# ivanacollg/MPC_CollisionAvoidance

Measured on AMD Instinct MI355X. Metric: batched SQP-RTI solves/sec (USV, N=40 horizon, 10 obstacles), higher is better.
Workload: dtype f64

## Files before the change

mpc_collisionavoidance_amd/csrc/params.hpp:

```cpp
#pragma once

namespace usv {

constexpr int LANES = 16;
constexpr int KMAX = 32;

struct DevSpec {
    double Hc[LANES * LANES];
    double He[LANES * LANES];
    double Mc[LANES * LANES];
    double Me[LANES * LANES];
    double lb[LANES], ub[LANES];
    int has_b[LANES];
    int boxpack;
    int boxpack_ok;
    int box_dense;
    int aux_dense4;
    int box_slot[LANES];
    int box_step[LANES];
    int slot_var[LANES];
    int slot_is[LANES];
    double uh[KMAX];
    double lsl[KMAX], lsu[KMAX];
    double zl[KMAX], zu[KMAX], Zl[KMAX], Zu[KMAX];
// ... 96 lines not shown
    double *u;
    const double *x0;
    const double *yref;
    const double *yref_e;
    const double *p;
    const double *lh;
    double *sl, *su;
    double *pi;
    int *status;
    int *qp_iter;
    int *qp_status;
    double *res;
    double *obs_tmin;
    int *fail_count;
    double *nlp_res;
    int *sqp_iter;
    int *sqp_state;
    int *sqp_running;
    double *ws;
    int *queue;
    int *epoch;
    int *redo;
    int redo_words;
    const int *perm_cur;
    const int *inv_next;
    int tick;
    double *lam_out, *t_out;
    int nlam;
    int *susp_count;
    int *susp_list;
    double *susp_rec;
    int handover_iter;
    int *co_ctl;
};

}
```

mpc_collisionavoidance_amd/csrc/qp_ipm.hpp:

```cpp
#pragma once
#include "lanes.hpp"
#include "params.hpp"
#include "sfor.hpp"

#pragma clang fp contract(on)

namespace usv {

template <bool SOFTROW, bool MIXED = false>
struct RowCalc {
    double ll, lu, tl, tu, sl, su, lsl, lsu, tsl, tsu;
    double dl, du, zl, zu, Zl, Zu, bsl, bsu;
    bool act, soft;
    double rdl, rdu, rsl, rsu, rdsl, rdsu;
    USV_DEV bool is_soft() const
    {
        if constexpr (!SOFTROW) return false;
        else if constexpr (MIXED) return soft;
        else return true;
    }
    double itl, itu, itsl, itsu;
    double Gl, Gu, iDl, iDu, rhol, rhou;
    double ml, mu, msl, msu;
    double dll, dlu, dtl, dtu, dsl, dsu, dlsl, dlsu, dtsl, dtsu;

    USV_DEV void neutral()
    {
        ll = lu = 0.0; tl = tu = 1.0; sl = su = 0.0; lsl = lsu = 0.0; tsl = tsu = 1.0;
        dl = -1.0; du = 1.0; zl = zu = 0.0; Zl = Zu = 1.0; bsl = bsu = -1.0;
        soft = SOFTROW && !MIXED;
    }
    USV_DEV void resid(double v)
    {
        rdl = v + sl - dl - tl;
        rdu = du - v + su - tu;
        lanes::frcp2(tl, tu, itl, itu);
        if constexpr (SOFTROW) {
            rsl = Zl * sl + zl - ll - lsl;
            rsu = Zu * su + zu - lu - lsu;
            rdsl = sl - bsl - tsl;
// ... 100 lines not shown
};

USV_DEV void obs_dist(double dx, double dy, double &d, double &ux, double &uy)
{
    const double d2 = dx * dx + dy * dy;
    const double id = lanes::frsqrt(d2);
    d = d2 * id;
    ux = dx * id; uy = dy * id;
}

template <class M, int KCH, bool SOFT, bool HDIAG, bool PACK, bool SOFTBOX = false, bool LDSWS = false, bool MERGE = false, bool AUXLDS = false,
          bool WIDE = false, int WW = 1, bool CPC = true>
struct QpIpm {
    static_assert(WW == 1 || (WIDE && (WW == 2 || WW == 4)), "several waves per instance: the wide mapping only");
    static_assert(!WIDE || (HDIAG && !AUXLDS), "the wide mapping works on every row layout of an OCP with a diagonal Hessian");
    static_assert(!MERGE || PACK, "merged row pass works on the packed layout");
    static_assert(!(AUXLDS && LDSWS), "with the whole workspace in LDS the aux plane is there already");
    static_assert(!PACK || KCH > 0, "box rows are packed into obstacle planes");
    static_assert(!(PACK && SOFTBOX), "soft state bounds are not packed");
    static constexpr int NX = M::NX, NU = M::NU, NZ = NX + NU;
    static constexpr int PXL = NU + M::IPX, PYL = NU + M::IPY;
    using MP = MatPack<M>;
    static_assert(NZ <= LANES, "one lane per variable of [u;x]");
    static_assert(NU <= 2, "the aux plane has room for two controls' r_g / l_u entries");
    static_assert(MP::NPK * 16 + 2 <= 256, "slot numbers of the exchange area are kept in one byte");
    using WL = WsLayout<M, KCH, SOFT, SOFTBOX>;
    enum : int { P_Z = WL::P_Z, P_AUX = WL::P_AUX, P_DZA = WL::P_DZA, P_DZ = WL::P_DZ, P_DX0 = WL::P_DX0, P_PB = WL::P_PB,
                 P_PI = WL::P_PI, P_BLL = WL::P_BLL, P_BLU = WL::P_BLU, P_BTL = WL::P_BTL, P_BTU = WL::P_BTU,
                 P_OBS = WL::P_OBS, P_LZU = WL::P_LZU, P_RB0 = WL::P_RB0, P_GQ = WL::P_GQ, P_MAT = WL::P_MAT,
                 P_BS = WL::P_BS };
    enum : int { AXL_ZX = WL::AXL_ZX, AXL_ZY = WL::AXL_ZY, AXL_RG = WL::AXL_RG, AXL_LU = WL::AXL_LU };
    static constexpr int OBSN = WL::OBSN;
    static constexpr int NPL = WL::NPT;

    static constexpr bool out_unit(int j) { return ((M::OUT_UNIT >> j) & 1u) != 0u; }
    static constexpr unsigned XMASK = (1u << NX) - 1u, ZMASK = (1u << NZ) - 1u;
    static constexpr unsigned NONUNIT = XMASK & ~(unsigned)M::OUT_UNIT;

    template <unsigned MASK, class F>
    USV_DEV static void groups_of_four(F f)
    {
        constexpr int n = __builtin_popcount(MASK);
        sfor<0, (n + 3) / 4>([&](auto g) {
            constexpr int i0 = 4 * g, m = (n - i0 < 4) ? n - i0 : 4;
            constexpr int j0 = MP::nth(MASK, i0), j1 = m > 1 ? MP::nth(MASK, i0 + 1) : 0, j2 = m > 2 ? MP::nth(MASK, i0 + 2) : 0,
                          j3 = m > 3 ? MP::nth(MASK, i0 + 3) : 0;
            f(std::integral_constant<int, m>{}, std::integral_constant<int, j0>{}, std::integral_constant<int, j1>{},
              std::integral_constant<int, j2>{}, std::integral_constant<int, j3>{});
        });
    }
    template <unsigned MASK, int KOFF, class FA>
    USV_DEV static void dot_lanes(double &acc, double b, FA a_of)
    {
        groups_of_four<MASK>([&](auto m, auto j0, auto j1, auto j2, auto j3) {
            if constexpr (m == 4) lanes::fma_bc4<KOFF + j0, KOFF + j1, KOFF + j2, KOFF + j3>(acc, b, a_of(j0), b, a_of(j1), b, a_of(j2), b, a_of(j3));
            else if constexpr (m == 3) lanes::fma_bc3<KOFF + j0, KOFF + j1, KOFF + j2>(acc, b, a_of(j0), b, a_of(j1), b, a_of(j2));
            else if constexpr (m == 2) lanes::fma_bc2<KOFF + j0, KOFF + j1>(acc, b, a_of(j0), b, a_of(j1));
            else lanes::fma_bc<KOFF + j0>(acc, b, a_of(j0));
        });
    }
    template <unsigned MASK, int K, class FB, class FA>
    USV_DEV static void dot_col(double &acc, FB b_of, FA a_of)
    {
        groups_of_four<MASK>([&](auto m, auto j0, auto j1, auto j2, auto j3) {
            if constexpr (m == 4) lanes::fma_bc4<K, K, K, K>(acc, b_of(j0), a_of(j0), b_of(j1), a_of(j1), b_of(j2), a_of(j2), b_of(j3), a_of(j3));
            else if constexpr (m == 3) lanes::fma_bc3<K, K, K>(acc, b_of(j0), a_of(j0), b_of(j1), a_of(j1), b_of(j2), a_of(j2));
            else if constexpr (m == 2) lanes::fma_bc2<K, K>(acc, b_of(j0), a_of(j0), b_of(j1), a_of(j1));
            else lanes::fma_bc<K>(acc, b_of(j0), a_of(j0));
        });
    }

    using BoxRow = RowCalc<SOFTBOX, SOFTBOX>;
    using ObsRow = RowCalc<SOFT, SOFT && MERGE>;
    struct WideMap {
        static constexpr int at(int plane)
        {
            if (!PACK) return plane < WL::P_RB0 ? plane : ((SOFTBOX && plane >= WL::P_BS && plane < WL::P_BS + 6) ? WL::P_RB0 + (plane - WL::P_BS) : -1);
            return plane < WL::P_BLL ? plane : (plane >= WL::P_OBS && plane < WL::P_RB0 ? plane - 4 : -1);
        }
    };
    static constexpr int NPLW = (WIDE && LDSWS) ? WL::P_RB0 - (PACK ? 4 : 0) + (SOFTBOX ? 6 : 0) : WL::NPT;
    using Planes = std::conditional_t<WIDE && LDSWS, lanes::PlanesLdsMapped<WideMap>, std::conditional_t<LDSWS, lanes::PlanesLds, lanes::Planes>>;

    const DevPtrs &P;
    const DevSpec &S;
    double rbscale;
    int Kn, nB, itmax;
    bool pstat;
    bool keep;
    int lane, N;
    long g, b;
    unsigned voff;
    unsigned loff;
    bool live;
    unsigned auxoff;
    int auxstride;
    bool auxlive;
    long stage_stride;
    unsigned stage_bytes;
    bool xlane, ulane, valid, isPX, isPY;
    bool ounit;
    static constexpr unsigned CMASK = MP::col_mask();
    static constexpr int NCOL = __builtin_popcount(CMASK);
    static constexpr int ZSLOT = MP::NPK * 16, OSLOT = ZSLOT + 1;
    using XP = lanes::Xpose<MP::NPK * 16 + 2, (WIDE ? WW : 4), WIDE>;
    unsigned rowtab[(NX + 3) / 4], coltab[(NCOL + 3) / 4];
    bool selfone;
    bool isslot, isdense, anydense;
    bool slot_u;
    int bsrc, bstep, ssrc;
    bool hasb;
    static constexpr int KC = KCH > 0 ? KCH : 1;
    enum : int {
        ST_LB = 0, ST_UB, ST_HDS, ST_HDT, ST_UH, ST_OX = ST_UH + KC, ST_OY = ST_OX + KC, ST_LH = ST_OY + KC, ST_SOFT = ST_LH + KC,
        ST_ZL = ST_SOFT, ST_ZU = ST_ZL + (SOFT ? KC : 0), ST_QL = ST_ZU + (SOFT ? KC : 0), ST_QU = ST_QL + (SOFT ? KC : 0),
        ST_BSL = ST_QU + (SOFT ? KC : 0), ST_BSU = ST_BSL + (SOFT ? KC : 0), ST_BOX = ST_BSU + (SOFT ? KC : 0),
// ... 106 lines not shown
        }
        auxoff = 0; auxstride = 0; auxlive = false;
        if constexpr (AUXLDS) {
            const int nd4 = lanes::uniform(S.aux_dense4);
            constexpr int ZB = KCH > 0 ? 2 : 0;
            int slot = lane < nd4 ? lane : -1;
            if constexpr (KCH > 0) slot = lane == AXL_ZX ? nd4 : (lane == AXL_ZY ? nd4 + 1 : slot);
            sfor<0, NU>([&](auto l) {
                slot = lane == AXL_RG - l ? nd4 + ZB + l : slot;
                slot = lane == AXL_LU - l ? nd4 + ZB + NU + l : slot;
            });
            auxlive = slot >= 0;
            auxstride = (nd4 + ZB + 2 * NU) * lanes::WAVE_ROWS;
            auxoff = (unsigned)((slot > 0 ? slot : 0) * lanes::WAVE_ROWS) + lanes::wave_row();
        }
        g = 0; b = 0;
        live = lds_row >= 0;
        loff = (unsigned)((lds_row > 0 ? lds_row : 0) * (N + 1) * NPLW * LANES + lane);
        if constexpr (KCH > 0) sfor<0, KCH>([&](auto c) { c_ox[c] = 0.0; c_oy[c] = 0.0; c_lh[c] = 0.0; });
        bind(g_, true);
        if constexpr (KCH > 0 && SOFT) {
            sfor<0, KCH>([&](auto c) {
                const int i = c * LANES + lane;
                const int ii = i < S.K ? i : 0;
                c_zl[c] = S.zl[ii]; c_zu[c] = S.zu[ii];
                c_Zl[c] = i < S.K ? S.Zl[ii] : 1.0; c_Zu[c] = i < S.K ? S.Zu[ii] : 1.0;
                c_bsl[c] = S.lsl[ii]; c_bsu[c] = S.lsu[ii];
            });
        }
    }

    USV_DEV void bind(long gn, bool sel)
    {
        g = sel ? gn : g;
        const long gi = g < nB ? g : (long)nB - 1;
        const long bn = P.perm ? (long)P.perm[gi] : gi;
        b = sel ? bn : b;
        voff = sel ? lanes::Planes::lane_offset(g, NPL, lane) : voff;
        if constexpr (KCH > 0) {
            sfor<0, KCH>([&](auto c) {
                const int i = c * LANES + lane;
                const int ii = i < Kn ? i : 0;
                const double ox = P.p[(long)b * (N + 1) * 2 * Kn + 2 * ii], oy = P.p[(long)b * (N + 1) * 2 * Kn + 2 * ii + 1];
                const double lh = P.lh[(long)b * N * Kn + ii];
                c_ox[c] = sel ? ox : c_ox[c]; c_oy[c] = sel ? oy : c_oy[c]; c_lh[c] = sel ? lh : c_lh[c];
            });
        }
    }

    USV_DEV lanes::Planes wsg(int k) const { return lanes::Planes(P.ws + (long)k * stage_stride, stage_bytes, voff); }
    USV_DEV Planes ws(int k) const
    {
        if constexpr (LDSWS) return Planes(loff + (unsigned)(k * NPLW * LANES), live);
        else return wsg(k);
    }
    USV_DEV double aux_ld(int k, const Planes &W) const
    {
        if constexpr (AUXLDS) return lanes::dyn_lds()[auxoff + (unsigned)(k * auxstride)];
        else return W.ld(P_AUX);
    }
    USV_DEV void aux_st(int k, const Planes &W, double v) const
    {
        if constexpr (AUXLDS) { if (auxlive) lanes::dyn_lds()[auxoff + (unsigned)(k * auxstride)] = v; }
        else W.st(P_AUX, v);
    }
    USV_DEV double zbar(int k) const
    {
        if (ulane) return (k < N) ? P.u[((long)b * N + k) * NU + lane] : 0.0;
        if (xlane) return P.x[((long)b * (N + 1) + k) * NX + (lane - NU)];
        return 0.0;
    }

    USV_DEV void box_data(int k, BoxRow &r) const
    {
        const bool stage_ok = ulane ? (k < N) : (k >= 1 && k < N);
        r.act = valid && hasb && stage_ok;
        r.dl = r.act ? lbv : -1.0;
        r.du = r.act ? ubv : 1.0;
        if constexpr (SOFTBOX) {
// ... 83 lines not shown
    }
    USV_DEV double pos_sel(double zbx, double zby) const { return isPX ? zbx : (isPY ? zby : 0.0); }
    USV_DEV void mat_issue(int k, double *pk) const
    {
        const Planes W = ws(k);
        sfor<0, MP::NPK>([&](auto q) { pk[q] = W.ld(P_MAT + q); });
    }
    USV_DEV void mat_put(const double *pk) const
    {
        sfor<0, MP::NPK>([&](auto q) { XP::put(16 * q + lane, pk[q]); });
        XP::sync();
    }
    USV_DEV void mat_unpack(const double *pk, double *bat) const
    {
        mat_put(pk);
        sfor<0, NX>([&](auto j) {
            if constexpr (out_unit(j)) bat[j] = 0.0;
            else bat[j] = XP::get((int)((rowtab[j / 4] >> (8 * (j % 4))) & 0xffu));
        });
    }
    USV_DEV double mat_apply(const double *pk, double dz, double acc) const
    {
        mat_put(pk);
        double v[NCOL];
        sfor<0, NCOL>([&](auto ci) { v[ci] = XP::get((int)((coltab[ci / 4] >> (8 * (ci % 4))) & 0xffu)); });
        dot_lanes<CMASK, 0>(acc, dz, [&](auto c) { return v[__builtin_popcount(CMASK & ((1u << c) - 1u))]; });
        return acc + (selfone ? dz : 0.0);
    }
    USV_DEV static double obs_dot(double cx, double cy, double vec)
    {
        return cx * lanes::bcast<PXL>(vec) + cy * lanes::bcast<PYL>(vec);
    }

    USV_DEV bool init(bool sel)
    {
        const bool wr = sel && !keep && (!(WIDE && !LDSWS) || live);
        double bad0 = 0.0;
        for (int k = 0; k <= N; k++) {
            const Planes W = ws(k);
            const double zb = zbar(k);
            if constexpr (LDSWS && !WIDE) {
                const lanes::Planes G = wsg(k);
                const double gq = G.ld(P_GQ), rb = (k < N) ? G.ld(P_RB0) : 0.0;
                double mpk[MP::NPK];
                if (k < N) sfor<0, MP::NPK>([&](auto q) { mpk[q] = G.ld(P_MAT + q); });
                if (wr) {
                    W.st(P_GQ, gq);
                    if (k < N) {
                        W.st(P_RB0, rb);
                        sfor<0, MP::NPK>([&](auto q) { W.st(P_MAT + q, mpk[q]); });
                    }
                }
            }
            if (wr) {
                W.st(P_Z, zb);
                if (k == 0) W.st(P_DX0, xlane ? P.x0[(long)b * NX + (lane - NU)] : 0.0);
            }
            BoxRow r;
            r.neutral();
            box_data(k, r);
            const double v0 = r.act ? zb : 0.0;
            r.tl = fmax(v0 - r.dl, S.thr0); r.tu = fmax(r.du - v0, S.thr0);
            r.ll = S.mu0 / r.tl; r.lu = S.mu0 / r.tu;
            if constexpr (SOFTBOX) {
                if (r.soft) {
                    r.tsl = fmax(0.0 - r.bsl, S.thr0); r.tsu = fmax(0.0 - r.bsu, S.thr0);
                    r.lsl = S.mu0 / r.tsl; r.lsu = S.mu0 / r.tsu;
                }
            }
            double pk[4], dv = 0.0;
            if constexpr (PACK) dv = box_pack(r, pk);
            else if (wr) box_store(W, r);
            const double zbx = KCH > 0 ? lanes::bcast<PXL>(zb) : 0.0, zby = KCH > 0 ? lanes::bcast<PYL>(zb) : 0.0;
            const double aux = aux_compose(dv, zbx, zby, 0.0, 0.0);
            if (wr) aux_st(k, W, aux);
            if constexpr (KCH > 0) {
                sfor<0, KCH>([&](auto c) {
                    ObsRow o;
                    double cx, cy, raw[3];
                    o.neutral();
                    obs_raw<c>(k, raw);
                    obs_geom<c>(k, zbx, zby, raw, o, cx, cy);
                    o.tl = fmax(0.0 - o.dl, S.thr0); o.tu = fmax(o.du - 0.0, S.thr0);
                    o.ll = S.mu0 / o.tl; o.lu = S.mu0 / o.tu;
                    if constexpr (SOFT) {
                        o.tsl = fmax(0.0 - o.bsl, S.thr0); o.tsu = fmax(0.0 - o.bsu, S.thr0);
                        o.lsl = S.mu0 / o.tsl; o.lsu = S.mu0 / o.tsu;
                    }
                    if (wr) obs_store(W, c, o, (PACK && c == KCH - 1) ? pk : nullptr);
                    if constexpr (!SOFT) {
                        if (k == 0) {
                            const double e0 = xlane ? P.x0[(long)b * NX + (lane - NU)] - zb : 0.0;
                            double d, ux, uy;
                            obs_dist(zbx - raw[0], zby - raw[1], d, ux, uy);
                            const double v0 = ux * lanes::bcast<PXL>(e0) + uy * lanes::bcast<PYL>(e0);
                            const bool row = c * LANES + lane < Kn;
                            const double tol = S.tol_ineq;
                            bad0 = (row && (raw[2] - d - v0 > tol || d + v0 - c_uh[c] > tol)) ? 1.0 : bad0;
                        }
                    }
                });
            }
        }
        return lanes::gmax(bad0) > 0.5;
    }

    struct Norms { double rg, rb, rd, rm, musum, nan; };

    template <bool CP = false, class R>
    USV_DEV static void chain(R &r, double v, bool corr, double w_aff, double sigmu, double &Gh, double &gam, double so = 1.0)
    {
        r.resid(v);
        r.targets_pred();
        r.reduce(Gh, gam);
        if (corr) {
            r.expand(w_aff);
            r.template targets_corr<CP>(sigmu, so);
            r.reduce(Gh, gam);
        }
    }

    struct StageIn {
        double z, aux, rb, dz, dza, gq, pb;
        double lzu[NU];
        double box[4];
        double bxs[SOFTBOX ? 6 : 1];
        double obs[KCH > 0 ? KCH : 1][OBSN];
        double raw[KCH > 0 ? KCH : 1][3];
    };
    enum : int { SW_BACK_A = 0, SW_FWD_A = 1, SW_BACK_B = 2, SW_FWD_B = 3 };

    template <int SW>
    USV_DEV void load_in(int k, StageIn &in) const
    {
        const Planes W = ws(k);
// ... 1107 lines not shown
            load_in<SW_FWD_A>(k, in);
            const double zbx = aux_zx(in.aux), zby = aux_zy(in.aux);
            double *L = P.lam_out + ((long)b * (N + 1) + k) * nlam, *T = P.t_out + ((long)b * (N + 1) + k) * nlam;
            BoxRow br;
            box_from(in, k, br);
            if (real && br.act) {
                const int i = S.box_pos[lane];
                L[i] = br.ll; L[nrow + i] = br.lu; T[i] = br.tl; T[nrow + i] = br.tu;
                if constexpr (SOFTBOX) {
                    if (br.soft) {
                        const int j = S.sbx_pos[lane];
                        L[ns0 + j] = br.lsl; L[ns0 + ns + j] = br.lsu; T[ns0 + j] = br.tsl; T[ns0 + ns + j] = br.tsu;
                    }
                }
            }
            if constexpr (KCH > 0) {
                sfor<0, KCH>([&](auto c) {
                    ObsRow o;
                    double cx, cy;
                    obs_from<c, false>(in, k, zbx, zby, o, cx, cy);
                    const int i = S.nbu + S.nbx + c * LANES + lane;
                    if (real && o.act) {
                        L[i] = o.ll; L[nrow + i] = o.lu; T[i] = o.tl; T[nrow + i] = o.tu;
                        if constexpr (SOFT) {
                            const int j = S.nsbx + c * LANES + lane;
                            L[ns0 + j] = o.lsl; L[ns0 + ns + j] = o.lsu; T[ns0 + j] = o.tsl; T[ns0 + ns + j] = o.tsu;
                        }
                    }
                });
            }
        }
    }

    USV_DEV void finish(bool fin, bool real, int status, int iters, int phase)
    {
        const bool ok = (status == 0 || status == 1);
        const bool out = fin && real;
        const bool share = P.epoch != nullptr;
        double tmin = 1e300;
        for (int k = 0; k <= N; k++) {
            const Planes W = ws(k);
            const double z = W.ld(P_Z);
            if constexpr (KCH > 0) {
                if (k >= 1 && k < N) {
                    sfor<0, KCH>([&](auto c) {
                        const double tl = W.ld(P_OBS + c * OBSN + 2);
                        tmin = (c * LANES + lane < Kn) ? fmin(tmin, tl) : tmin;
                    });
                }
            }
            if constexpr (LDSWS) {
                if (out) {
                    const lanes::Planes G = wsg(k);
                    G.st(P_AUX, W.ld(P_AUX));
                    G.st(P_PI, W.ld(P_PI));
                    if constexpr (!PACK) {
                        G.st(P_BLL, W.ld(P_BLL)); G.st(P_BLU, W.ld(P_BLU)); G.st(P_BTL, W.ld(P_BTL)); G.st(P_BTU, W.ld(P_BTU));
                        if constexpr (SOFTBOX) sfor<0, 6>([&](auto e) { G.st(P_BS + e, W.ld(P_BS + e)); });
                    }
                    if constexpr (KCH > 0) sfor<0, KCH * OBSN>([&](auto e) { G.st(P_OBS + e, W.ld(P_OBS + e)); });
                }
            }
            if constexpr (AUXLDS) {
                if (out) W.st(P_AUX, aux_ld(k, W));
            }
            if (out) {
                if (share) {
                    if (ok && xlane) lanes::st_shared(&P.x[((long)b * (N + 1) + k) * NX + (lane - NU)], z);
                    if (ok && ulane && k < N) lanes::st_shared(&P.u[((long)b * N + k) * NU + lane], z);
                } else {
                    if (ok && xlane) P.x[((long)b * (N + 1) + k) * NX + (lane - NU)] = z;
                    if (ok && ulane && k < N) P.u[((long)b * N + k) * NU + lane] = z;
                }
                if (k >= 1 && xlane && P.pi) P.pi[((long)b * N + (k - 1)) * NX + (lane - NU)] = W.ld(P_PI);
            }
            if constexpr (KCH > 0 && SOFT) {
                if (k >= 1 && k < N) {
                    sfor<0, KCH>([&](auto c) {
                        const int i = c * LANES + lane;
                        if (out && i < Kn && P.sl) {
                            const int p0 = P_OBS + c * OBSN;
                            P.sl[((long)b * N + k) * Kn + i] = W.ld(p0 + 4);
                            P.su[((long)b * N + k) * Kn + i] = W.ld(p0 + 5);
                        }
                    });
                } else if (k == 0) {
                    const double aux = aux_ld(0, W);
                    const double zbx = aux_zx(aux), zby = aux_zy(aux);
                    const double e0 = z - pos_sel(zbx, zby);
                    sfor<0, KCH>([&](auto c) {
                        const int i = c * LANES + lane;
                        double raw[3], d, ux, uy;
                        obs_raw<c>(0, raw);
                        obs_dist(zbx - raw[0], zby - raw[1], d, ux, uy);
                        const double v0 = ux * lanes::bcast<PXL>(e0) + uy * lanes::bcast<PYL>(e0);
                        double a = fmax(c_bsl[c], raw[2] - d - v0), q = fmax(c_bsu[c], d + v0 - c_uh[c]);
                        if (c_Zl[c] > 0.0) a = fmax(a, -c_zl[c] / c_Zl[c]);
// ... 58 lines not shown
        const bool co = P.co_ctl != nullptr;
        if (co) lanes::release_agent();
        if (sel && lane == 0) {
            const int slot = lanes::fetch_add(P.susp_count);
            if (co) lanes::publish(P.susp_list + slot, (int)g);
            else P.susp_list[slot] = (int)g;
        }
    }

    USV_DEV void solve(int phase, int queue0)
    {
        bool frozen = false;
        keep = false;
        const bool resume = phase == 3;
        if (resume) phase = 0;
        if (phase > 0) {
            const bool real0 = g < nB;
            frozen = !real0 || P.sqp_state[b] >= 0;
            if (!lanes::wave_any(!frozen)) return;
            double nr[4];
            nlp_residual(phase == 1, nr);
            if (!frozen) {
                const bool conv = nr[0] <= S.nlp_tol[0] && nr[1] <= S.nlp_tol[1] && nr[2] <= S.nlp_tol[2] && nr[3] <= S.nlp_tol[3];
                if (lane == 0) {
                    P.nlp_res[b * 4 + 0] = nr[0]; P.nlp_res[b * 4 + 1] = nr[1];
                    P.nlp_res[b * 4 + 2] = nr[2]; P.nlp_res[b * 4 + 3] = nr[3];
                    if (conv) P.sqp_state[b] = 0;
                }
                frozen = conv;
            }
            if (!lanes::wave_any(!frozen)) return;
        }
        keep = frozen;
        const bool bad0 = resume ? false : init(true);
        rbscale = 1.0;
        const bool own = WIDE ? true : live;
        bool real = g < nB && !frozen && live;
        bool done = frozen || !own;
        bool pend = false;
        bool fresh = false;
        bool late = bad0 && !frozen && own;
        int status = late ? 4 : 1, iters = 0, it = 0;
        done = done || late;
        Norms nm;
        double a_prev = 0.0, sig_prev = 0.0;
        const double nc = (double)S.nc;
        const bool refill = phase == 0 && queue0 >= 0;
        const bool cpc = CPC && lanes::uniform(S.cpc) != 0;
        if constexpr (HAS_CPC) { so_prv = 1.0; so_cur = 1.0; }
        if constexpr (WIDE) {
            if (resume) {
                copy_in();
                const double *r = P.susp_rec + 4 * b;
                const double r3 = r[3];
                a_prev = r[0]; sig_prev = r[1]; rbscale = r[2];
                it = (int)fabs(r3);
                if constexpr (CPC) so_prv = (r3 < 0.0) ? 0.0 : 1.0;
                iters = it;
                pend = true;
            }
        }
        const int hand_it = (CAN_SUSPEND && phase == 0 && P.susp_count != nullptr) ? P.handover_iter : 0;
        for (;;) {
            backward<true>(nm, 0.0, pend && !done, a_prev, sig_prev);
            bool fin = late;
            if (!done) {
                if (real && lane == 0) {
                    P.res[b * 4 + 0] = nm.rg; P.res[b * 4 + 1] = nm.rb; P.res[b * 4 + 2] = nm.rd; P.res[b * 4 + 3] = nm.rm;
                }
                iters = it;
                if (nm.nan != nm.nan) { status = 3; fin = true; }
                else if (nm.rg <= S.tol_stat && nm.rb <= S.tol_eq && nm.rd <= S.tol_ineq && nm.rm <= S.tol_comp) {
                    status = 0; fin = true;
                } else if (it >= itmax) { status = 1; fin = true; }
            }
            done = done || fin;
            late = false;
            if (lanes::wave_any(fin)) {
                finish(fin, real, status, iters, phase);
                real = fin ? false : real;
                bool took = false;
                if (refill) {
                    int gn = 0;
                    if constexpr (WIDE) {
                        if (fin && lanes::block_row() == 0u && lane == 0) gn = queue0 + lanes::fetch_add(P.queue);
                        gn = xwave_first_i(lanes::wave_first_i(gn));
                    } else {
                        if (fin && lane == 0) gn = queue0 + lanes::fetch_add(P.queue);
                        gn = lanes::bcast_i<0>(gn);
                    }
                    const bool take = fin && gn < nB;
                    took = take;
                    if (lanes::wave_any(take)) {
                        if constexpr (WW > 1) lanes::block_sync();
                        bind((long)gn, take);
                        const bool bad = init(take) && take;
                        real = take ? (WIDE ? live : true) : real;
                        done = take ? bad : done;
                        late = bad;
                        fresh = take;
                        pend = take ? false : pend;
                        rbscale = take ? 1.0 : rbscale;
                        it = take ? 0 : it;
                        iters = take ? 0 : iters;
                        status = take ? (bad ? 4 : 1) : status;
                        if constexpr (HAS_CPC) { const double sp = so_prv; so_prv = take ? 1.0 : sp; }
                        if constexpr (!LDSWS && !WIDE) voff = take ? stage_bytes + (unsigned)(lane * 8) : voff;
                    }
                }
                if constexpr (!LDSWS && !WIDE) {
                    if (phase == 0) voff = (fin && !took) ? stage_bytes + (unsigned)(lane * 8) : voff;
                }
            }
            if (!lanes::wave_any(!done || late)) break;
            const bool run = !done && !fresh;
            const double mu = nc > 0.0 ? nm.musum / nc : 0.0;
            double a_aff = 1.0, S1 = 0.0, S2 = 0.0, a = 1.0, d1 = 0.0, d2 = 0.0;
            forward<false>(0.0, a_aff, S1, S2);
            double sigmu = 0.0, mu_aff = 0.0;
            if (nc > 0.0) {
                mu_aff = (nm.musum + a_aff * S1 + a_aff * a_aff * S2) / nc;
                const double sg = mu_aff / mu;
                sigmu = sg * sg * sg * mu;
            }
            if constexpr (HAS_CPC) so_cur = 1.0;
            backward<false>(nm, sigmu, false, 0.0, 0.0);
            forward<true>(sigmu, a, d1, d2);
            if constexpr (HAS_CPC) {
                const double mu_pc = nc > 0.0 ? (nm.musum + a * d1 + a * a * d2) / nc : 0.0;
                const bool refuse = cpc && run && nc > 0.0 && mu_pc > S.cpc_factor * mu_aff;
                if (lanes::wave_any(refuse)) {
                    so_cur = refuse ? 0.0 : 1.0;
                    double a2 = 1.0;
                    backward<false>(nm, sigmu, false, 0.0, 0.0);
                    forward<true>(sigmu, a2, d1, d2);
                    a = refuse ? a2 : a;
                }
            }
            if (run && a < S.alpha_min) { status = 2; done = true; late = true; iters = it; }
            a_prev = run ? a * ((1.0 - a) * 0.99 + a * 0.9999999) : a_prev;
            sig_prev = run ? sigmu : sig_prev;
            if constexpr (HAS_CPC) { const double sp = so_prv, sc = so_cur; so_prv = run ? sc : sp; }
            pend = run ? true : pend;
            it = run ? it + 1 : it;
            if constexpr (!LDSWS && !WIDE) voff = fresh ? lanes::Planes::lane_offset(g, NPL, lane) : voff;
            fresh = false;
            if constexpr (CAN_SUSPEND) {
                if (hand_it > 0) {
                    const bool drained = !refill || lanes::observe(P.queue) >= nB - queue0;
                    const bool sus = drained && !done && real && it >= hand_it;
                    if (lanes::wave_any(sus)) {
                        suspend(sus, it, a_prev, sig_prev);
                        done = done || sus;
                        real = sus ? false : real;
                        voff = sus ? stage_bytes + (unsigned)(lane * 8) : voff;
                    }
                }
            }
        }
    }
};

}

#pragma clang fp contract(fast)
```

mpc_collisionavoidance_amd/csrc/usvmpc.hip:

```cpp
#ifndef USV_PART
#define USV_PART -1
#endif
#define USV_MAIN (USV_PART <= 0)

#include "gfx950/lanes.hpp"

#include "guidance.hpp"
#include "host_spec.hpp"
#include "linearize.hpp"
#include "models.hpp"
#include "obstacle_tracks.hpp"
#include "qp_ipm.hpp"
#include "sim.hpp"
#include "cond_launch.hpp"
#ifdef USV_GEN_MODEL_HEADER
#include USV_GEN_MODEL_HEADER
#endif

#include <algorithm>
#include <cstdint>
#include <cstdio>
#include <cstring>
#include <mutex>
#include <string>
// ... 932 lines not shown
    const void *f = (const void *)kern;
    hipFuncAttributes fa;
    int nb = 0;
    if (f == nullptr || hipFuncGetAttributes(&fa, f) != hipSuccess || fa.sharedSizeBytes + dyn > 160u * 1024u || set_dynamic_lds(f, dyn) != hipSuccess ||
        hipOccupancyMaxActiveBlocksPerMultiprocessor(&nb, f, block, dyn) != hipSuccess)
        return 0;
    return nb;
}

void co_release(usvmpc_handle *h)
{
    if (h->co_stream) { (void)hipStreamSynchronize(h->co_stream); (void)hipStreamDestroy(h->co_stream); }
    if (h->ev_co_pre) (void)hipEventDestroy(h->ev_co_pre);
    if (h->ev_co_end) (void)hipEventDestroy(h->ev_co_end);
    dev_free(h, h->d_co_ctl, (size_t)usvmpc_handle::RING * 8 * sizeof(int));
    h->co_stream = nullptr; h->ev_co_pre = nullptr; h->ev_co_end = nullptr; h->d_co_ctl = nullptr;
    h->co_ready = false;
}

bool co_prepare(usvmpc_handle *h)
{
    if (h->co_ready) return true;
    int prio_least = 0, prio_greatest = 0;
    const bool ok = hipDeviceGetStreamPriorityRange(&prio_least, &prio_greatest) == hipSuccess &&
                    hipStreamCreateWithPriority(&h->co_stream, hipStreamNonBlocking, prio_least) == hipSuccess &&
                    hipEventCreateWithFlags(&h->ev_co_pre, hipEventDisableTiming) == hipSuccess &&
                    hipEventCreateWithFlags(&h->ev_co_end, hipEventDisableTiming) == hipSuccess &&
                    dev_alloc(h, &h->d_co_ctl, (size_t)usvmpc_handle::RING * 8, true) == 0;
    if (ok) h->co_ready = true;
    else { co_release(h); h->handover_co = 0; (void)hipGetLastError(); }
    return ok;
}

int launch_qp(usvmpc_handle *h, const Kernels &k, int phase)
{
    const int qp_block = 64;
    const long qp_groups = h->Bp;
    hipEvent_t *ev = h->ev[h->nsolves % usvmpc_handle::RING];
    const long lds_inst = (long)(h->N + 1) * h->spec.npt * 128;
    h->last_wide = 0;
    h->ptrs.susp_count = nullptr; h->ptrs.susp_list = nullptr; h->ptrs.susp_rec = nullptr; h->ptrs.handover_iter = 0; h->ptrs.co_ctl = nullptr;
    if (k.wide_lds4 != nullptr && phase == 0 && h->wide_mode != 0 && h->wide_waves != 1 && h->ncu > 0) {
        const size_t pl = (size_t)(h->N + 1) * (size_t)k.nplw * 128;
        const size_t b4 = pl + (size_t)16 * k.ex_lds * 128 + 128, x4 = (size_t)16 * k.ex_hbm * 128 + 128;
        const long win_bytes = (long)std::min(h->N + 1, 16) * h->Bp * h->spec.npt * 128;
        if (h->wide4_cap == 0) h->wide4_cap = blocks_per_cu(k.wide_lds4, 4 * qp_block, b4) > 0 ? (long)h->ncu : -1;
        if (h->wide4_cap < 0 && h->wide4_hbm_cap == 0)
            h->wide4_hbm_cap = (win_bytes < (1L << 32) && blocks_per_cu(k.wide_hbm4, 4 * qp_block, x4) > 0) ? (long)h->ncu : -1;
        const bool lds = h->wide4_cap > 0;
        long cap = lds ? h->wide4_cap : h->wide4_hbm_cap;
        if (cap > 0 && h->max_waves > 0) cap = std::max<long>(1, std::min(cap, h->max_waves / 4));
        const long reach = (h->dynamic_rows && h->N >= 40) ? 2 * cap : cap;
        const bool hard_many = !k.soft && k.kch == 1 && h->K >= 8 && h->N >= 40 && (long)h->B <= cap;
        if (cap > 0 && (h->wide_waves == 4 || ((k.soft || k.kch == 2) && (long)h->B <= reach) || hard_many)) {
            long nw = (long)h->B;
            int q0 = -1;
            if (h->dynamic_rows && nw > cap) { nw = cap; q0 = (int)nw; }
            if (q0 >= 0) HIP_TRY(h, hipMemsetAsync(h->ptrs.queue, 0, sizeof(int), h->stream));
            hipLaunchKernelGGL(lds ? k.wide_lds4 : k.wide_hbm4, dim3((unsigned)nw), dim3(4 * qp_block), lds ? b4 : x4, h->stream, h->ptrs, nw, phase, q0, 1);
            h->last_wide = 4;
            return 0;
        }
    }
    if (k.wide_lds1 != nullptr && h->wide_mode != 0 && h->ncu > 0) {
        if (phase == 0) {
            const size_t bytes = (size_t)(h->N + 1) * (size_t)k.nplw * 128 + (size_t)4 * k.ex_lds * 128;
            if (h->wide_cap == 0) {
                const int nb = blocks_per_cu(k.wide_lds1, qp_block, bytes);
                h->wide_cap = nb > 0 ? (long)std::min(nb, 4) * h->ncu : -1;
// ... 1500 lines not shown
```

Measured before the change: 985,300.

## Batch init and finish stage loads in groups of four to overlap memory latency

For the streamed (non-LDS, non-wide) QP path, init and finish now issue loads for four horizon stages at once, settle them, then run the per-stage compute and stores, so global-memory latency overlaps across stages instead of serialising per stage. bind now uses a real branch instead of selects, avoiding loads for lanes that are not rebinding. It also adds compile-time-gated cycle-counter instrumentation for turnover phases. Costs are more live registers per wave and some restructuring of the finish path, including moving the AUXLDS aux copy.

Measured after the change: 986,700 (median of 3 runs). About the same (+0.1%).

```diff
diff --git a/mpc_collisionavoidance_amd/csrc/params.hpp b/mpc_collisionavoidance_amd/csrc/params.hpp
--- a/mpc_collisionavoidance_amd/csrc/params.hpp
+++ b/mpc_collisionavoidance_amd/csrc/params.hpp
@@ -152,6 +152,9 @@
     double *susp_rec;
     int handover_iter;
     int *co_ctl;
+#if defined(USV_TURNOVER_TIMING)
+    unsigned long long *tt;
+#endif
 };
 
 }
diff --git a/mpc_collisionavoidance_amd/csrc/qp_ipm.hpp b/mpc_collisionavoidance_amd/csrc/qp_ipm.hpp
--- a/mpc_collisionavoidance_amd/csrc/qp_ipm.hpp
+++ b/mpc_collisionavoidance_amd/csrc/qp_ipm.hpp
@@ -6,6 +6,19 @@
 #pragma clang fp contract(on)
 
 namespace usv {
+
+enum : int { TT_OTHER = 0, TT_FINISH, TT_BIND, TT_INIT, TT_BACK_A, TT_FWD_A, TT_BACK_B, TT_FWD_B, TT_FIN1, TT_FIN2, TT_FIN3, TT_FIN4, TT_INITS, TT_WAVES, TT_N };
+#if defined(USV_TURNOVER_TIMING) && defined(__HIPCC__)
+#define USV_TT_BEGIN() tt_last = __builtin_readcyclecounter()
+#define USV_TT(slot) tt_mark(slot)
+#define USV_TT_ADD(slot, n) tt_acc[slot] += (unsigned long long)(n)
+#define USV_TT_END() tt_flush()
+#else
+#define USV_TT_BEGIN()
+#define USV_TT(slot)
+#define USV_TT_ADD(slot, n)
+#define USV_TT_END()
+#endif
 
 template <bool SOFTROW, bool MIXED = false>
 struct RowCalc {
@@ -172,6 +185,8 @@
     enum : int { AXL_ZX = WL::AXL_ZX, AXL_ZY = WL::AXL_ZY, AXL_RG = WL::AXL_RG, AXL_LU = WL::AXL_LU };
     static constexpr int OBSN = WL::OBSN;
     static constexpr int NPL = WL::NPT;
+    static constexpr bool STREAMED = !LDSWS && !WIDE;
+    static constexpr int FB = 4;
 
     static constexpr bool out_unit(int j) { return ((M::OUT_UNIT >> j) & 1u) != 0u; }
     static constexpr unsigned XMASK = (1u << NX) - 1u, ZMASK = (1u << NZ) - 1u;
@@ -222,6 +237,21 @@
     static constexpr int NPLW = (WIDE && LDSWS) ? WL::P_RB0 - (PACK ? 4 : 0) + (SOFTBOX ? 6 : 0) : WL::NPT;
     using Planes = std::conditional_t<WIDE && LDSWS, lanes::PlanesLdsMapped<WideMap>, std::conditional_t<LDSWS, lanes::PlanesLds, lanes::Planes>>;
 
+#if defined(USV_TURNOVER_TIMING) && defined(__HIPCC__)
+    unsigned long long tt_last = 0, tt_acc[TT_N] = {};
+    USV_DEV void tt_mark(int slot)
+    {
+        const unsigned long long t = __builtin_readcyclecounter();
+        tt_acc[slot] += t - tt_last;
+        tt_last = t;
+    }
+    USV_DEV void tt_flush()
+    {
+        tt_acc[TT_WAVES] = 1;
+        if (lanes::wave_lane() == 0u && P.tt != nullptr)
+            sfor<0, TT_N>([&](auto i) { atomicAdd(P.tt + i, tt_acc[i]); });
+    }
+#endif
     const DevPtrs &P;
     const DevSpec &S;
     double rbscale;
@@ -394,19 +424,19 @@
 
     USV_DEV void bind(long gn, bool sel)
     {
-        g = sel ? gn : g;
-        const long gi = g < nB ? g : (long)nB - 1;
-        const long bn = P.perm ? (long)P.perm[gi] : gi;
-        b = sel ? bn : b;
-        voff = sel ? lanes::Planes::lane_offset(g, NPL, lane) : voff;
-        if constexpr (KCH > 0) {
-            sfor<0, KCH>([&](auto c) {
-                const int i = c * LANES + lane;
-                const int ii = i < Kn ? i : 0;
-                const double ox = P.p[(long)b * (N + 1) * 2 * Kn + 2 * ii], oy = P.p[(long)b * (N + 1) * 2 * Kn + 2 * ii + 1];
-                const double lh = P.lh[(long)b * N * Kn + ii];
-                c_ox[c] = sel ? ox : c_ox[c]; c_oy[c] = sel ? oy : c_oy[c]; c_lh[c] = sel ? lh : c_lh[c];
-            });
+        if (sel) {
+            g = gn;
+            const long gi = g < nB ? g : (long)nB - 1;
+            b = P.perm ? (long)P.perm[gi] : gi;
+            voff = lanes::Planes::lane_offset(g, NPL, lane);
+            if constexpr (KCH > 0) {
+                sfor<0, KCH>([&](auto c) {
+                    const int i = c * LANES + lane;
+                    const int ii = i < Kn ? i : 0;
+                    c_ox[c] = P.p[(long)b * (N + 1) * 2 * Kn + 2 * ii]; c_oy[c] = P.p[(long)b * (N + 1) * 2 * Kn + 2 * ii + 1];
+                    c_lh[c] = P.lh[(long)b * N * Kn + ii];
+                });
+            }
         }
     }
 
@@ -556,75 +586,116 @@
         return cx * lanes::bcast<PXL>(vec) + cy * lanes::bcast<PYL>(vec);
     }
 
+    USV_DEV static void landed(double &v) { lanes::settle(v); }
+    struct InitIn {
+        double zb, x0;
+        double raw[KC][3];
+    };
+    template <int IB>
+    USV_DEV void init_load(int kb, bool sel, InitIn *in) const
+    {
+        sfor<0, IB>([&](auto j) {
+            in[j].zb = 0.0; in[j].x0 = 0.0;
+            sfor<0, KC>([&](auto c) { in[j].raw[c][0] = 0.0; in[j].raw[c][1] = 0.0; in[j].raw[c][2] = 0.0; });
+        });
+        if (sel) {
+            sfor<0, IB>([&](auto j) {
+                const int k = kb + j;
+                if (k <= N) {
+                    const int ku = k < N ? k : N - 1;
+                    const double *pz = ulane ? P.u + ((long)b * N + ku) * NU + lane : P.x + ((long)b * (N + 1) + k) * NX + (lane - NU);
+                    if (valid) in[j].zb = *pz;
+                    if (k == 0 && xlane) in[j].x0 = P.x0[(long)b * NX + (lane - NU)];
+                    if constexpr (KCH > 0) {
+                        if (!pstat) sfor<0, KCH>([&](auto c) { obs_raw<c>(k, in[j].raw[c]); });
+                    }
+                }
+            });
+        }
+    }
+    USV_DEV void init_stage(int k, bool wr, const InitIn &in, double thr0, double mu0, double tol, double &bad0) const
+    {
+        const Planes W = ws(k);
+        const double zb = (ulane && k == N) ? 0.0 : in.zb;
+        if constexpr (LDSWS && !WIDE) {
+            const lanes::Planes G = wsg(k);
+            const double gq = G.ld(P_GQ), rb = (k < N) ? G.ld(P_RB0) : 0.0;
+            double mpk[MP::NPK];
+            if (k < N) sfor<0, MP::NPK>([&](auto q) { mpk[q] = G.ld(P_MAT + q); });
+            if (wr) {
+                W.st(P_GQ, gq);
+                if (k < N) {
+                    W.st(P_RB0, rb);
+                    sfor<0, MP::NPK>([&](auto q) { W.st(P_MAT + q, mpk[q]); });
+                }
+            }
+        }
+        if (wr) {
+            W.st(P_Z, zb);
+            if (k == 0) W.st(P_DX0, in.x0);
+        }
+        BoxRow r;
+        r.neutral();
+        box_data(k, r);
+        const double v0 = r.act ? zb : 0.0;
+        r.tl = fmax(v0 - r.dl, thr0); r.tu = fmax(r.du - v0, thr0);
+        r.ll = mu0 / r.tl; r.lu = mu0 / r.tu;
+        if constexpr (SOFTBOX) {
+            if (r.soft) {
+                r.tsl = fmax(0.0 - r.bsl, thr0); r.tsu = fmax(0.0 - r.bsu, thr0);
+                r.lsl = mu0 / r.tsl; r.lsu = mu0 / r.tsu;
+            }
+        }
+        double pk[4], dv = 0.0;
+        if constexpr (PACK) dv = box_pack(r, pk);
+        else if (wr) box_store(W, r);
+        const double zbx = KCH > 0 ? lanes::bcast<PXL>(zb) : 0.0, zby = KCH > 0 ? lanes::bcast<PYL>(zb) : 0.0;
+        const double aux = aux_compose(dv, zbx, zby, 0.0, 0.0);
+        if (wr) aux_st(k, W, aux);
+        if constexpr (KCH > 0) {
+            sfor<0, KCH>([&](auto c) {
+                ObsRow o;
+                double cx, cy, raw[3];
+                o.neutral();
+                if (pstat) obs_raw<c>(k, raw);
+                else { raw[0] = in.raw[c][0]; raw[1] = in.raw[c][1]; raw[2] = in.raw[c][2]; }
+                obs_geom<c>(k, zbx, zby, raw, o, cx, cy);
+                o.tl = fmax(0.0 - o.dl, thr0); o.tu = fmax(o.du - 0.0, thr0);
+                o.ll = mu0 / o.tl; o.lu = mu0 / o.tu;
+                if constexpr (SOFT) {
+                    o.tsl = fmax(0.0 - o.bsl, thr0); o.tsu = fmax(0.0 - o.bsu, thr0);
+                    o.lsl = mu0 / o.tsl; o.lsu = mu0 / o.tsu;
+                }
+                if (wr) obs_store(W, c, o, (PACK && c == KCH - 1) ? pk : nullptr);
+                if constexpr (!SOFT) {
+                    if (k == 0) {
+                        const double e0 = xlane ? in.x0 - zb : 0.0;
+                        double d, ux, uy;
+                        obs_dist(zbx - raw[0], zby - raw[1], d, ux, uy);
+                        const double v0 = ux * lanes::bcast<PXL>(e0) + uy * lanes::bcast<PYL>(e0);
+                        const bool row = c * LANES + lane < Kn;
+                        bad0 = (row && (raw[2] - d - v0 > tol || d + v0 - c_uh[c] > tol)) ? 1.0 : bad0;
+                    }
+                }
+            });
+        }
+    }
     USV_DEV bool init(bool sel)
     {
         const bool wr = sel && !keep && (!(WIDE && !LDSWS) || live);
         double bad0 = 0.0;
-        for (int k = 0; k <= N; k++) {
-            const Planes W = ws(k);
-            const double zb = zbar(k);
-            if constexpr (LDSWS && !WIDE) {
-                const lanes::Planes G = wsg(k);
-                const double gq = G.ld(P_GQ), rb = (k < N) ? G.ld(P_RB0) : 0.0;
-                double mpk[MP::NPK];
-                if (k < N) sfor<0, MP::NPK>([&](auto q) { mpk[q] = G.ld(P_MAT + q); });
-                if (wr) {
-                    W.st(P_GQ, gq);
-                    if (k < N) {
-                        W.st(P_RB0, rb);
-                        sfor<0, MP::NPK>([&](auto q) { W.st(P_MAT + q, mpk[q]); });
-                    }
-                }
-            }
-            if (wr) {
-                W.st(P_Z, zb);
-                if (k == 0) W.st(P_DX0, xlane ? P.x0[(long)b * NX + (lane - NU)] : 0.0);
-            }
-            BoxRow r;
-            r.neutral();
-            box_data(k, r);
-            const double v0 = r.act ? zb : 0.0;
-            r.tl = fmax(v0 - r.dl, S.thr0); r.tu = fmax(r.du - v0, S.thr0);
-            r.ll = S.mu0 / r.tl; r.lu = S.mu0 / r.tu;
-            if constexpr (SOFTBOX) {
-                if (r.soft) {
-                    r.tsl = fmax(0.0 - r.bsl, S.thr0); r.tsu = fmax(0.0 - r.bsu, S.thr0);
-                    r.lsl = S.mu0 / r.tsl; r.lsu = S.mu0 / r.tsu;
-                }
-            }
-            double pk[4], dv = 0.0;
-            if constexpr (PACK) dv = box_pack(r, pk);
-            else if (wr) box_store(W, r);
-            const double zbx = KCH > 0 ? lanes::bcast<PXL>(zb) : 0.0, zby = KCH > 0 ? lanes::bcast<PYL>(zb) : 0.0;
-            const double aux = aux_compose(dv, zbx, zby, 0.0, 0.0);
-            if (wr) aux_st(k, W, aux);
-            if constexpr (KCH > 0) {
-                sfor<0, KCH>([&](auto c) {
-                    ObsRow o;
-                    double cx, cy, raw[3];
-                    o.neutral();
-                    obs_raw<c>(k, raw);
-                    obs_geom<c>(k, zbx, zby, raw, o, cx, cy);
-                    o.tl = fmax(0.0 - o.dl, S.thr0); o.tu = fmax(o.du - 0.0, S.thr0);
-                    o.ll = S.mu0 / o.tl; o.lu = S.mu0 / o.tu;
-                    if constexpr (SOFT) {
-                        o.tsl = fmax(0.0 - o.bsl, S.thr0); o.tsu = fmax(0.0 - o.bsu, S.thr0);
-                        o.lsl = S.mu0 / o.tsl; o.lsu = S.mu0 / o.tsu;
-                    }
-                    if (wr) obs_store(W, c, o, (PACK && c == KCH - 1) ? pk : nullptr);
-                    if constexpr (!SOFT) {
-                        if (k == 0) {
-                            const double e0 = xlane ? P.x0[(long)b * NX + (lane - NU)] - zb : 0.0;
-                            double d, ux, uy;
-                            obs_dist(zbx - raw[0], zby - raw[1], d, ux, uy);
-                            const double v0 = ux * lanes::bcast<PXL>(e0) + uy * lanes::bcast<PYL>(e0);
-                            const bool row = c * LANES + lane < Kn;
-                            const double tol = S.tol_ineq;
-                            bad0 = (row && (raw[2] - d - v0 > tol || d + v0 - c_uh[c] > tol)) ? 1.0 : bad0;
-                        }
-                    }
+        const double thr0 = S.thr0, mu0 = S.mu0, tol = S.tol_ineq;
+        constexpr int IB = STREAMED ? FB : 1;
+        for (int kb = 0; kb <= N; kb += IB) {
+            InitIn in[IB];
+            init_load<IB>(kb, sel, in);
+            if constexpr (STREAMED) {
+                sfor<0, IB>([&](auto j) {
+                    landed(in[j].zb); landed(in[j].x0);
+                    sfor<0, KC>([&](auto c) { landed(in[j].raw[c][0]); landed(in[j].raw[c][1]); landed(in[j].raw[c][2]); });
                 });
             }
+            sfor<0, IB>([&](auto j) { if (kb + j <= N) init_stage(kb + j, wr, in[j], thr0, mu0, tol, bad0); });
         }
         return lanes::gmax(bad0) > 0.5;
     }
@@ -1798,13 +1869,98 @@
         }
     }
 
+    struct FinIn {
+        double z, pi, tl[KC];
+        double s[SOFT ? 2 * KC : 1];
+    };
+    USV_DEV void finish_load(int k, FinIn &in) const
+    {
+        const Planes W = ws(k);
+        in.z = W.ld(P_Z);
+        if (k >= 1 && P.pi) in.pi = W.ld(P_PI);
+        if constexpr (KCH > 0) {
+            if (k >= 1 && k < N) {
+                sfor<0, KCH>([&](auto c) {
+                    in.tl[c] = W.ld(P_OBS + c * OBSN + 2);
+                    if constexpr (SOFT) {
+                        if (P.sl) { in.s[2 * c] = W.ld(P_OBS + c * OBSN + 4); in.s[2 * c + 1] = W.ld(P_OBS + c * OBSN + 5); }
+                    }
+                });
+            } else if (SOFT && k == 0) in.s[0] = aux_ld(0, W);
+        }
+    }
+    USV_DEV void finish_store(int k, const FinIn &in, bool out, bool ok, bool share, double &tmin) const
+    {
+        const Planes W = ws(k);
+        const double z = in.z;
+        if constexpr (KCH > 0) {
+            if (k >= 1 && k < N) sfor<0, KCH>([&](auto c) { tmin = (c * LANES + lane < Kn) ? fmin(tmin, in.tl[c]) : tmin; });
+        }
+        if constexpr (AUXLDS) {
+            if (out) W.st(P_AUX, aux_ld(k, W));
+        }
+        if (out) {
+            if (share) {
+                if (ok && xlane) lanes::st_shared(&P.x[((long)b * (N + 1) + k) * NX + (lane - NU)], z);
+                if (ok && ulane && k < N) lanes::st_shared(&P.u[((long)b * N + k) * NU + lane], z);
+            } else {
+                if (ok && xlane) P.x[((long)b * (N + 1) + k) * NX + (lane - NU)] = z;
+                if (ok && ulane && k < N) P.u[((long)b * N + k) * NU + lane] = z;
+            }
+            if (k >= 1 && xlane && P.pi) P.pi[((long)b * N + (k - 1)) * NX + (lane - NU)] = in.pi;
+        }
+        if constexpr (KCH > 0 && SOFT) {
+            if (k >= 1 && k < N) {
+                sfor<0, KCH>([&](auto c) {
+                    const int i = c * LANES + lane;
+                    if (out && i < Kn && P.sl) {
+                        P.sl[((long)b * N + k) * Kn + i] = in.s[2 * c];
+                        P.su[((long)b * N + k) * Kn + i] = in.s[2 * c + 1];
+                    }
+                });
+            } else if (k == 0) {
+                const double aux = in.s[0];
+                const double zbx = aux_zx(aux), zby = aux_zy(aux);
+                const double e0 = z - pos_sel(zbx, zby);
+                sfor<0, KCH>([&](auto c) {
+                    const int i = c * LANES + lane;
+                    double raw[3], d, ux, uy;
+                    obs_raw<c>(0, raw);
+                    obs_dist(zbx - raw[0], zby - raw[1], d, ux, uy);
+                    const double v0 = ux * lanes::bcast<PXL>(e0) + uy * lanes::bcast<PYL>(e0);
+                    double a = fmax(c_bsl[c], raw[2] - d - v0), q = fmax(c_bsu[c], d + v0 - c_uh[c]);
+                    if (c_Zl[c] > 0.0) a = fmax(a, -c_zl[c] / c_Zl[c]);
+                    if (c_Zu[c] > 0.0) q = fmax(q, -c_zu[c] / c_Zu[c]);
+                    if (out && i < Kn && P.sl) {
+                        P.sl[(long)b * N * Kn + i] = a;
+                        P.su[(long)b * N * Kn + i] = q;
+                    }
+                });
+            }
+        }
+    }
+
     USV_DEV void finish(bool fin, bool real, int status, int iters, int phase)
     {
         const bool ok = (status == 0 || status == 1);
         const bool out = fin && real;
         const bool share = P.epoch != nullptr;
         double tmin = 1e300;
-        for (int k = 0; k <= N; k++) {
+        if constexpr (STREAMED) {
+            const unsigned voff_row = voff;
+            voff = out ? voff : stage_bytes + (unsigned)(lane * 8);
+            for (int kb = 0; kb <= N; kb += FB) {
+                FinIn in[FB] = {};
+                sfor<0, FB>([&](auto j) { if (kb + j <= N) finish_load(kb + j, in[j]); });
+                sfor<0, FB>([&](auto j) {
+                    landed(in[j].z); landed(in[j].pi);
+                    sfor<0, KC>([&](auto c) { landed(in[j].tl[c]); });
+                    sfor<0, (SOFT ? 2 * KC : 1)>([&](auto e) { landed(in[j].s[e]); });
+                });
+                sfor<0, FB>([&](auto j) { if (kb + j <= N) finish_store(kb + j, in[j], out, ok, share, tmin); });
+            }
+            voff = voff_row;
+        } else for (int k = 0; k <= N; k++) {
             const Planes W = ws(k);
             const double z = W.ld(P_Z);
             if constexpr (KCH > 0) {
@@ -1826,9 +1982,6 @@
                     }
                     if constexpr (KCH > 0) sfor<0, KCH * OBSN>([&](auto e) { G.st(P_OBS + e, W.ld(P_OBS + e)); });
                 }
-            }
-            if constexpr (AUXLDS) {
-                if (out) W.st(P_AUX, aux_ld(k, W));
             }
             if (out) {
                 if (share) {
@@ -1953,7 +2106,10 @@
             if (!lanes::wave_any(!frozen)) return;
         }
         keep = frozen;
+        USV_TT_BEGIN();
         const bool bad0 = resume ? false : init(true);
+        USV_TT(TT_INIT);
+        USV_TT_ADD(TT_INITS, 1);
         rbscale = 1.0;
         const bool own = WIDE ? true : live;
         bool real = g < nB && !frozen && live;
@@ -1983,7 +2139,9 @@
         }
         const int hand_it = (CAN_SUSPEND && phase == 0 && P.susp_count != nullptr) ? P.handover_iter : 0;
         for (;;) {
+            USV_TT(TT_OTHER);
             backward<true>(nm, 0.0, pend && !done, a_prev, sig_prev);
+            USV_TT(TT_BACK_A);
             bool fin = late;
             if (!done) {
                 if (real && lane == 0) {
@@ -1998,7 +2156,13 @@
             done = done || fin;
             late = false;
             if (lanes::wave_any(fin)) {
+                USV_TT(TT_OTHER);
                 finish(fin, real, status, iters, phase);
+                USV_TT(TT_FINISH);
+                USV_TT_ADD(TT_FIN1, __popcll(__ballot(fin && lane == 0)) == 1);
+                USV_TT_ADD(TT_FIN2, __popcll(__ballot(fin && lane == 0)) == 2);
+                USV_TT_ADD(TT_FIN3, __popcll(__ballot(fin && lane == 0)) == 3);
+                USV_TT_ADD(TT_FIN4, __popcll(__ballot(fin && lane == 0)) >= 4);
                 real = fin ? false : real;
                 bool took = false;
                 if (refill) {
@@ -2015,7 +2179,10 @@
                     if (lanes::wave_any(take)) {
                         if constexpr (WW > 1) lanes::block_sync();
                         bind((long)gn, take);
+                        USV_TT(TT_BIND);
                         const bool bad = init(take) && take;
+                        USV_TT(TT_INIT);
+                        USV_TT_ADD(TT_INITS, 1);
                         real = take ? (WIDE ? live : true) : real;
                         done = take ? bad : done;
                         late = bad;
@@ -2032,12 +2199,15 @@
                 if constexpr (!LDSWS && !WIDE) {
                     if (phase == 0) voff = (fin && !took) ? stage_bytes + (unsigned)(lane * 8) : voff;
                 }
+                USV_TT(TT_BIND);
             }
             if (!lanes::wave_any(!done || late)) break;
             const bool run = !done && !fresh;
             const double mu = nc > 0.0 ? nm.musum / nc : 0.0;
             double a_aff = 1.0, S1 = 0.0, S2 = 0.0, a = 1.0, d1 = 0.0, d2 = 0.0;
+            USV_TT(TT_OTHER);
             forward<false>(0.0, a_aff, S1, S2);
+            USV_TT(TT_FWD_A);
             double sigmu = 0.0, mu_aff = 0.0;
             if (nc > 0.0) {
                 mu_aff = (nm.musum + a_aff * S1 + a_aff * a_aff * S2) / nc;
@@ -2045,16 +2215,22 @@
                 sigmu = sg * sg * sg * mu;
             }
             if constexpr (HAS_CPC) so_cur = 1.0;
+            USV_TT(TT_OTHER);
             backward<false>(nm, sigmu, false, 0.0, 0.0);
+            USV_TT(TT_BACK_B);
             forward<true>(sigmu, a, d1, d2);
+            USV_TT(TT_FWD_B);
             if constexpr (HAS_CPC) {
                 const double mu_pc = nc > 0.0 ? (nm.musum + a * d1 + a * a * d2) / nc : 0.0;
                 const bool refuse = cpc && run && nc > 0.0 && mu_pc > S.cpc_factor * mu_aff;
                 if (lanes::wave_any(refuse)) {
                     so_cur = refuse ? 0.0 : 1.0;
                     double a2 = 1.0;
+                    USV_TT(TT_OTHER);
                     backward<false>(nm, sigmu, false, 0.0, 0.0);
+                    USV_TT(TT_BACK_B);
                     forward<true>(sigmu, a2, d1, d2);
+                    USV_TT(TT_FWD_B);
                     a = refuse ? a2 : a;
                 }
             }
@@ -2079,6 +2255,8 @@
                 }
             }
         }
+        USV_TT(TT_OTHER);
+        USV_TT_END();
     }
 };
 
diff --git a/mpc_collisionavoidance_amd/csrc/usvmpc.hip b/mpc_collisionavoidance_amd/csrc/usvmpc.hip
--- a/mpc_collisionavoidance_amd/csrc/usvmpc.hip
+++ b/mpc_collisionavoidance_amd/csrc/usvmpc.hip
@@ -988,9 +988,26 @@
     return ok;
 }
 
+#if defined(USV_TURNOVER_TIMING)
+static unsigned long long *g_turnover_ticks = nullptr;
+extern "C" int usvmpc_debug_turnover_ticks(unsigned long long *out, int reset)
+{
+    if (!g_turnover_ticks) {
+        if (hipMalloc((void **)&g_turnover_ticks, TT_N * sizeof(unsigned long long)) != hipSuccess) return -1;
+        reset = 1;
+    }
+    if (hipDeviceSynchronize() != hipSuccess) return -1;
+    if (out && !reset && hipMemcpy(out, g_turnover_ticks, TT_N * sizeof(unsigned long long), hipMemcpyDeviceToHost) != hipSuccess) return -1;
+    if (reset && hipMemset(g_turnover_ticks, 0, TT_N * sizeof(unsigned long long)) != hipSuccess) return -1;
+    return hipDeviceSynchronize() == hipSuccess ? 0 : -1;
+}
+#endif
 int launch_qp(usvmpc_handle *h, const Kernels &k, int phase)
 {
     const int qp_block = 64;
+#if defined(USV_TURNOVER_TIMING)
+    h->ptrs.tt = g_turnover_ticks;
+#endif
     const long qp_groups = h->Bp;
     hipEvent_t *ev = h->ev[h->nsolves % usvmpc_handle::RING];
     const long lds_inst = (long)(h->N + 1) * h->spec.npt * 128;
```
